# DCDmllm/AnyEdit

Measured on AMD Instinct MI355X. Metric: edited-images/sec @512x512, 50 DDIM steps, higher is better.
Workload: dtype bf16; 1 GPU; configs[1]: AnySD (SD-1.5 UNet in=8 + task embedding/expert adapters) 512x512 bf16, 50 DDIM steps, batch=4/GPU, 3-branch CFG (UNet batch 12); images_per_gpu=4, ddim_steps=50, cfg_branches=3, hip_graph=True, parallelism=dp1 (image-sharded, no data-path collective)

## Files before the change

### anyedit_amd/_lib.py

```python
import ctypes
import os

import torch

_HERE = os.path.dirname(os.path.abspath(__file__))
LIB_PATH = os.environ.get("AE_LIB_PATH") or os.path.join(_HERE, "libanyedit_hip.so")

c_void_p, c_int, c_long, c_float = ctypes.c_void_p, ctypes.c_int, ctypes.c_long, ctypes.c_float

SIGNATURES = {
    "ae_version": [],
    "ae_last_error": [],
    "ae_device_arch": [ctypes.c_char_p, c_int],
    "ae_device_info": [ctypes.POINTER(c_int), ctypes.POINTER(c_long), ctypes.POINTER(c_int)],
    "ae_gemm_bf16": [c_void_p, c_long, c_void_p, c_long, c_int, c_void_p, c_long, c_void_p, c_long, c_int, c_int, c_int,
                     c_void_p, c_void_p, c_long, c_void_p, c_long, c_int, c_int, c_int, c_void_p, c_void_p],
    "ae_conv3x3_workspace_floats": [c_int, c_int, c_int, c_int, c_int, c_int, c_int],
    "ae_conv3x3_bf16": [c_void_p, c_void_p, c_void_p, c_void_p, c_long, c_void_p, c_void_p, c_int, c_int, c_int, c_int, c_int,
                        c_int, c_int, c_int, c_void_p, c_void_p, c_int, c_void_p],
    "ae_conv3x3_up2_bf16": [c_void_p, c_void_p, c_void_p, c_void_p, c_int, c_int, c_int, c_int, c_int, c_void_p, c_void_p],
    "ae_gemm_plan": [c_int] * 8 + [ctypes.POINTER(c_int)],
    "ae_conv3x3_plan": [c_int] * 11 + [ctypes.POINTER(c_int)],
    "ae_conv3x3_up2_plan": [c_int] * 6 + [ctypes.POINTER(c_int)],
    "ae_groupnorm_rows_per_chunk": [c_int, c_int],
    "ae_groupnorm_workspace_floats": [c_int, c_int, c_int, c_int],
    "ae_groupnorm_nhwc_bf16": [c_void_p, c_void_p, c_int, c_void_p, c_void_p, c_void_p, c_int, c_int, c_int, c_int, c_float,
                               c_int, c_void_p, c_void_p, c_void_p, c_void_p, c_void_p, c_void_p],
    "ae_layernorm_bf16": [c_void_p, c_void_p, c_void_p, c_void_p, c_int, c_int, c_float, c_void_p],
    "ae_attn_fwd_bf16": [c_void_p, c_void_p, c_void_p, c_void_p, c_int, c_int, c_int, c_int, c_int,
                         c_long, c_long, c_long, c_long, c_long, c_long, c_long, c_long, c_long, c_long, c_long, c_long,
                         c_float, c_void_p, c_void_p, c_int, c_int, c_void_p, c_void_p, c_int,
                         c_void_p, c_void_p, c_int, c_long, c_long, c_long, c_long, c_long, c_long, c_void_p, c_void_p, c_void_p,
                         c_void_p],
    "ae_attn_bwd_bf16": [c_void_p] * 10 + [c_int] * 5 + [c_long] * 21 + [c_float, c_void_p, c_int, c_void_p, c_void_p],
    "ae_attn_bwd_workspace_floats": [c_int] * 5,
    "ae_groupnorm_bwd_workspace_floats": [c_int, c_int, c_int, c_int],
    "ae_groupnorm_bwd_nhwc_bf16": [c_void_p, c_void_p, c_int, c_void_p, c_void_p, c_void_p, c_void_p, c_void_p, c_int, c_int, c_int,
                                   c_int, c_float, c_int, c_void_p, c_void_p, c_void_p, c_int, c_void_p],
    "ae_layernorm_bwd_bf16": [c_void_p, c_void_p, c_void_p, c_void_p, c_void_p, c_int, c_int, c_float, c_int, c_void_p],
    "ae_layernorm_param_grad_f32": [c_void_p, c_void_p, c_void_p, c_void_p, c_void_p, c_int, c_int, c_void_p],
    "ae_add_bf16": [c_void_p, c_void_p, c_void_p, c_long, c_void_p],
    "ae_axpy_bf16": [c_void_p, c_void_p, c_float, c_void_p, c_long, c_void_p],
    "ae_geglu_fwd_bf16": [c_void_p, c_void_p, c_long, c_int, c_void_p],
    "ae_geglu_bwd_bf16": [c_void_p, c_void_p, c_void_p, c_long, c_int, c_void_p],
    "ae_sumpool2x2_bf16": [c_void_p, c_void_p, c_int, c_int, c_int, c_int, c_void_p],
    "ae_colsum_bf16_f32": [c_void_p, c_void_p, c_int, c_int, c_long, c_void_p],
    "ae_mse_grad_f32": [c_void_p, c_void_p, c_void_p, c_long, c_float, c_void_p],
    "ae_adamw_f32": [c_void_p, c_void_p, c_void_p, c_void_p, c_long, c_float, c_float, c_float, c_float, c_float, c_int, c_float,
                     c_void_p],
    "ae_rowsum_f32": [c_void_p, c_void_p, c_int, c_long, c_void_p],
    "ae_scatter_add_rows_f32": [c_void_p, c_void_p, c_void_p, c_int, c_int, c_int, c_void_p],
    "ae_attn_fp8_workspace_bytes": [c_int, c_int, c_int, c_int, c_int],
    "ae_attn_fwd_fp8": [c_void_p, c_void_p, c_void_p, c_void_p, c_int, c_int, c_int, c_int, c_int] + [c_long] * 12 +
                       [c_float, c_void_p, c_void_p, c_int, c_int, c_void_p, c_long, c_void_p],
    "ae_ln_gemm_supported": [c_int, c_int, c_int, c_int],
    "ae_ln_gemm_bf16": [c_void_p, c_long, c_void_p, c_long, c_void_p, c_long, c_int, c_int, c_int, c_void_p, c_void_p, c_long, c_void_p, c_void_p,
                        c_float, c_int, c_void_p, c_void_p],
    "ae_gemm_ln_plan": [c_int, c_int, c_int, c_int, c_int],
    "ae_ff_fused_supported": [c_int, c_int, c_int],
    "ae_ff_fused_bf16": [c_void_p, c_long, c_void_p, c_void_p, c_float, c_void_p, c_long, c_void_p, c_void_p, c_void_p, c_void_p, c_long,
                         c_void_p, c_long, c_void_p, c_void_p, c_long, c_void_p, c_void_p, c_long, c_int, c_int, c_int, c_void_p],
    "ae_gemm_ln_bf16": [c_void_p, c_long, c_void_p, c_long, c_void_p, c_long, c_int, c_int, c_int, c_void_p, c_void_p, c_long, c_int, c_void_p,
                        c_void_p, c_int, c_void_p, c_float, c_void_p],
    "ae_task_gate_bwd": [c_void_p, c_void_p, c_void_p, c_void_p, c_int, c_int, c_int, c_void_p, c_void_p],
    "ae_task_gate_wgrad": [c_void_p, c_void_p, c_void_p, c_void_p, c_void_p, c_int, c_int, c_int, c_int, c_void_p, c_void_p, c_void_p],
    "ae_expert_kv_fwd": [c_void_p, c_void_p, c_void_p, c_void_p, c_int, c_int, c_int, c_int, c_int, c_void_p],
    "ae_expert_kv_dgrad_slices": [c_int],
    "ae_expert_kv_dgrad": [c_void_p, c_void_p, c_void_p, c_void_p, c_int, c_int, c_int, c_int, c_int, c_void_p, c_void_p],
    "ae_expert_kv_wgrad": [c_void_p, c_void_p, c_void_p, c_void_p, c_int, c_int, c_int, c_int, c_int, c_void_p],
    "ae_transpose_last2": [c_void_p, c_void_p, c_int, c_int, c_int, c_int, c_int, c_int, c_void_p],
    "ae_concat_channels_bf16": [c_void_p, c_int, c_void_p, c_int, c_void_p, c_long, c_void_p],
    "ae_im2col3x3_c8_bf16": [c_void_p, c_void_p, c_int, c_int, c_int, c_void_p],
    "ae_split_channels_bf16": [c_void_p, c_int, c_int, c_void_p, c_void_p, c_long, c_int, c_int, c_void_p],
    "ae_timestep_embedding": [c_void_p, c_void_p, c_void_p, c_void_p, c_int, c_int, c_float, c_void_p],
    "ae_ddim_step_f32": [c_void_p, c_void_p, c_void_p, c_void_p, c_void_p, c_void_p, c_long, c_int, c_float, c_float, c_float,
                         c_float, c_float, c_float, c_float, c_float, c_void_p],
# ... 121 lines not shown
```

### anyedit_amd/csrc/common.hpp

```cpp
#pragma once
#include <hip/hip_runtime.h>
#include <stdint.h>

typedef uint16_t bf16_t;
typedef __attribute__((ext_vector_type(8))) __bf16 bf16x8_t;
typedef __attribute__((ext_vector_type(4))) float f32x4;
typedef __attribute__((ext_vector_type(2))) float f32x2;
typedef __attribute__((ext_vector_type(4))) uint32_t u32x4;
typedef __attribute__((ext_vector_type(2))) uint32_t u32x2;

#define AE_OK 0
#define AE_ERR_ARG -1
#define AE_ERR_LAUNCH -2
#define AE_ERR_UNSUPPORTED -3

void ae_set_error(const char* fmt, ...);
int ae_check_launch(const char* what);
int ae_launch_colstats(const uint16_t* x, long ld, int M, int N, float* out, hipStream_t stream);

int ae_rowpanel_fold_covers(int M, int N, int K, int epilogue, int mode);
int ae_rowpanel_fold_launch(const void* A, long lda, const void* W, long ldw, void* C, long ldc, int M, int N, int K, const float* bias, const void* residual,
                            long ldr, int epilogue, float* rowstats_out, const float* ln_stats, int ln_parts, const float* ln_colsum, float ln_eps, void* stream);

#define AE_REQUIRE(cond, ...)                 \
// ... 37 lines not shown
}
__device__ __forceinline__ float erf_as_f(float z) {
    const float az = __builtin_fabsf(z);
    const float t = __builtin_amdgcn_rcpf(__builtin_fmaf(0.3275911f, az, 1.0f));
    float poly = __builtin_fmaf(1.061405429f, t, -1.453152027f);
    poly = __builtin_fmaf(poly, t, 1.421413741f);
    poly = __builtin_fmaf(poly, t, -0.284496736f);
    poly = __builtin_fmaf(poly, t, 0.254829592f);
    poly *= t;
    const float e = __builtin_amdgcn_exp2f(-1.4426950408889634f * az * az);
    const float r = __builtin_fmaf(-poly, e, 1.0f);
    return __builtin_copysignf(r, z);
}
#ifndef AE_GELU_POLY
#define AE_GELU_POLY 0
#endif
__device__ __forceinline__ float gelu_w_poly_f(float x) {
    const float ax = __builtin_fminf(__builtin_fabsf(x), 4.25f);
    const float t = __builtin_fmaf(ax * ax, 0.11072664707899094f, -1.0f);
    float p = __builtin_fmaf(0.004925727378576994f, t, -0.012811211869120598f);
    p = __builtin_fmaf(p, t, 0.017165469005703926f);
    p = __builtin_fmaf(p, t, -0.02821926586329937f);
    p = __builtin_fmaf(p, t, 0.05118509382009506f);
    p = __builtin_fmaf(p, t, -0.07870230078697205f);
    p = __builtin_fmaf(p, t, 0.11140184104442596f);
    p = __builtin_fmaf(p, t, -0.1615230143070221f);
    p = __builtin_fmaf(p, t, 0.33187076449394226f);
    return ax * p;
}
__device__ __forceinline__ float gelu_w_f(float x) {
    if (AE_GELU_POLY) return gelu_w_poly_f(x);
    const float ax = __builtin_fabsf(x);
    const float t = __builtin_amdgcn_rcpf(__builtin_fmaf(0.3275911f * 0.70710678118654752440f, ax, 1.0f));
    float poly = __builtin_fmaf(1.061405429f, t, -1.453152027f);
    poly = __builtin_fmaf(poly, t, 1.421413741f);
    poly = __builtin_fmaf(poly, t, -0.284496736f);
    poly = __builtin_fmaf(poly, t, 0.254829592f);
    poly *= t;
    const float e = __builtin_amdgcn_exp2f((-0.5f * 1.4426950408889634f) * ax * ax);
    return __builtin_fmaf(-poly, e, 1.0f);
}
#ifndef AE_GELU_OLD
#define AE_GELU_OLD 0
#endif
__device__ __forceinline__ float gelu_erf_f(float x) {
    if (AE_GELU_OLD) return 0.5f * x * (1.0f + erf_as_f(x * 0.70710678118654752440f));
    return 0.5f * __builtin_fmaf(__builtin_fabsf(x), gelu_w_f(x), x);
}
__device__ __forceinline__ float geglu_half_f(float a_half, float g) {
    if (AE_GELU_OLD) return (a_half + a_half) * gelu_erf_f(g);
    return a_half * __builtin_fmaf(__builtin_fabsf(g), gelu_w_f(g), g);
}

__device__ __forceinline__ int xcd_remap(int bid, int nblocks) {
    const int NX = 8;
    int xcd = bid % NX, j = bid / NX;
    int q = nblocks / NX, r = nblocks % NX;
    int base = (xcd < r) ? xcd * (q + 1) : r * (q + 1) + (xcd - r) * q;
    return base + j;
}

__device__ __forceinline__ void ae_dma16(__amdgpu_buffer_rsrc_t rs, int lds_byte, int voffset, int soffset = 0) {
#if defined(__HIP_DEVICE_COMPILE__)
    asm volatile("s_mov_b32 m0, %2\n\ts_nop 0\n\tbuffer_load_dwordx4 %0, %1, %3 offen lds" ::"v"(voffset), "s"(rs), "s"(lds_byte), "s"(soffset)
                 : "memory", "m0");
#endif
}

__device__ __forceinline__ float wave_reduce_sum(float v) {
#pragma unroll
    for (int o = 32; o > 0; o >>= 1) v += __shfl_xor(v, o, 64);
    return v;
}
__device__ __forceinline__ float wave_reduce_max(float v) {
#pragma unroll
    for (int o = 32; o > 0; o >>= 1) v = fmaxf(v, __shfl_xor(v, o, 64));
    return v;
}
```

### anyedit_amd/csrc/gemm_conv.hip

```cpp
#include "common.hpp"
#include <stdlib.h>
#include <string.h>
#include <type_traits>

namespace {

#ifndef AE_CONV_SPEC
#define AE_CONV_SPEC 1
#endif
#ifndef AE_XE_OCC
#define AE_XE_OCC 4
#endif
#ifndef AE_PP_LAB
#define AE_PP_LAB 0
#endif
#ifndef AE_PP_PRIO
#define AE_PP_PRIO 1
#endif
#ifndef AE_PP_DMA_FIRST
#define AE_PP_DMA_FIRST 0
#endif
constexpr int BK = 64;

enum { A_DENSE = 0, A_CONV3 = 1 };
enum { EPI_NONE = 0, EPI_GELU = 1, EPI_GEGLU = 2, EPI_SILU = 3, EPI_RELU = 4 };

struct GemmArgs {
    const bf16_t* A;
    const bf16_t* A2;
    const bf16_t* W;
    void* C;
    const float* bias;
    const bf16_t* res;
    const float* addvec;
    int M, N, K, Ksplit;
    long lda, lda2, ldw, ldc, ldr, ldav;
    int epi, out_f32, rows_per_batch;
    int H, Wd, Cin, CinPad, Ho, Wo, stride, ups;
    unsigned a_bytes, a2_bytes, w_bytes;
    int splitk;
    float* partial;
    float* colstats;
    int kmajor;
    int m_fast;
    int xe;
    float* rowstats;
    const float* ln_stats;
    const float* ln_colsum;
    int ln_parts;
    float ln_eps;
    int sub2;
};

__device__ __forceinline__ void lds_dma16(__amdgpu_buffer_rsrc_t rs, bf16_t* lds_dst, int voffset, int soffset = 0) {
#if defined(__HIP_DEVICE_COMPILE__)
    __builtin_amdgcn_raw_ptr_buffer_load_lds(rs, (__attribute__((address_space(3))) void*)lds_dst, 16, voffset, soffset, 0, 0);
#endif
}

#ifdef AE_GEMM_LAB
__device__ unsigned long long g_gemm_dbg[32];
#define GL_T(i) do { const unsigned long long t_ = __builtin_readcyclecounter(); if (lab_me) g_gemm_dbg[lab_base + (i)] += t_ - tlast; tlast = t_; } while (0)
#elif defined(AE_GEMM_TRACE)
constexpr int TR_K0 = 18, TR_T = 6;
__device__ unsigned long long g_pp_trace[8 * TR_T * 16];
#define GL_T(i) do { __builtin_amdgcn_sched_barrier(0); tr_t[(i)] = __builtin_readcyclecounter(); __builtin_amdgcn_sched_barrier(0); } while (0)
#else
#define GL_T(i)
#endif

constexpr int epilogue_passes(int FM, int bytes_per_frag_row, int lds_bytes) {
    for (int ps = 1; ps <= FM; ++ps)
        if (FM % ps == 0 && (FM / ps) * bytes_per_frag_row <= lds_bytes) return ps;
    return FM;
}

template <int BM, int BN, int AMODE, int WAVES_M = 2, int WAVES_N = 2, bool GLDS = false, int WAVES_K = 1, int STAGES = 2, bool CS = false, int LAB = 0, int WA = 0, int XE = 0>
__global__ __launch_bounds__(64 * WAVES_M * WAVES_N * WAVES_K, (XE == 2 && BM == 128 && BN == 128 && STAGES == 2) ? AE_XE_OCC : 0) void gemm_kernel(const GemmArgs p) {
    static_assert(XE == 0 || (AMODE == A_DENSE && WAVES_K == 1 && !CS && GLDS), "row statistics / LayerNorm fold: dense LDS-DMA instantiations, one K group, no column statistics");
    static_assert(XE != 1 || BN / WAVES_N == 64, "row statistics are emitted per 64-column slice = one wave tile's width");
    static_assert(STAGES == 2 || (GLDS && WAVES_K == 1), "the deep LDS ring exists only for the LDS-DMA loader");
    static_assert(!WA || (GLDS && STAGES == 2 && WAVES_K == 1), "operand-ahead is a variant of the two-stage LDS-DMA pipeline");
    static_assert(WA == 0 || WA == 1 || WA == 3 || WA == 4, "WA: 0 none, 1 weights two tiles ahead (three W stages), 3 ping-pong (two wave groups one barrier apart), 4 ping-pong over an activation slab per (channel chunk, ky)");
    static_assert(WA < 3 || 64 * WAVES_M * WAVES_N * WAVES_K == 512, "the ping-pong loops pair wave w with wave w + 4 (one SIMD's two waves)");
    static_assert(WA != 4 || (AMODE == A_CONV3 && GLDS && BM % 16 == 0), "the slab loop is a 3x3-convolution loop");
    static_assert(WAVES_K == 1, "one K group per block (the two-group form is removed: DESIGN.md, \"Built, measured, removed\")");
    constexpr int NT = 64 * WAVES_M * WAVES_N * WAVES_K;
    constexpr int WM = BM / WAVES_M, WN = BN / WAVES_N;
    constexpr int FM = WM / 16, FN = WN / 16;
    constexpr int A_CH = BM * 8 / NT, B_CH = BN * 8 / NT;
    static_assert((BM * 8) % NT == 0 && (BN * 8) % NT == 0, "tile / thread-count combination not supported");
    extern __shared__ __attribute__((aligned(16))) unsigned char smem_raw[];
    bf16_t* const smem = reinterpret_cast<bf16_t*>(smem_raw);
    bf16_t* sA = smem;
    bf16_t* sB = smem + (WA >= 3 ? 3 : STAGES) * BM * BK;

#ifndef AE_WAVE_SGPR
#define AE_WAVE_SGPR 1
#endif
    const int tid = threadIdx.x, lane = tid & 63, wave = AE_WAVE_SGPR ? __builtin_amdgcn_readfirstlane(tid >> 6) : tid >> 6;
#ifdef AE_GEMM_TRACE
    const bool tr_blk = blockIdx.x == gridDim.x / 2 && WA == 3;
    unsigned long long* const tr_lds = reinterpret_cast<unsigned long long*>(smem_raw + 152 * 1024);
    int tr_kt = -1;
    unsigned long long tr_t[16];
#pragma unroll
    for (int q = 0; q < 16; ++q) tr_t[q] = 0;
#endif
#ifdef AE_GEMM_LAB
    unsigned long long tlast = __builtin_readcyclecounter();
    const bool lab_me = blockIdx.x == gridDim.x / 2 && lane == 0 && (wave == 0 || wave == 4);
    const int lab_base = wave == 0 ? 0 : 16;
#endif
    const int wk = wave / (WAVES_M * WAVES_N), wmn = wave % (WAVES_M * WAVES_N);
    const int wm = wmn / WAVES_N, wn = wmn % WAVES_N;
    const int l15 = lane & 15, lg = lane >> 4;
    const int ntn = (p.N + BN - 1) / BN, ntm = (p.M + BM - 1) / BM;
    const int ntiles = ntm * ntn;
    const int split = blockIdx.x / ntiles;
    const int py = (AMODE == A_CONV3 && p.sub2) ? split >> 1 : 0, px = (AMODE == A_CONV3 && p.sub2) ? split & 1 : 0;
    const int tile = xcd_remap(blockIdx.x % ntiles, ntiles);
    const int m0 = (p.m_fast ? tile % ntm : tile / ntn) * BM, n0 = (p.m_fast ? tile / ntm : tile % ntn) * BN;

    long a_base[A_CH];
    int a_iy[A_CH], a_ix[A_CH];
#pragma unroll
    for (int i = 0; i < A_CH; ++i) {
        const int row = (tid + i * NT) >> 3;
        const int m = m0 + row;
        const int mc = min(m, p.M - 1);
        if (AMODE == A_DENSE) {
            a_base[i] = (long)mc;
            a_iy[i] = a_ix[i] = 0;
        } else {
            const int hw = p.Ho * p.Wo;
            const int b = mc / hw, rem = mc - b * hw;
            const int oy = rem / p.Wo, ox = rem - oy * p.Wo;
            a_base[i] = (long)b * p.H * p.Wd;
            a_iy[i] = (m < p.M) ? oy * p.stride - 1 : -100000;
            a_ix[i] = ox * p.stride - 1;
        }
    }
    long b_base[B_CH];
#pragma unroll
    for (int i = 0; i < B_CH; ++i) {
        const int row = (tid + i * NT) >> 3;
        b_base[i] = (long)min(n0 + row, p.N - 1) * p.ldw;
    }

    const __amdgpu_buffer_rsrc_t rsA = __builtin_amdgcn_make_buffer_rsrc(const_cast<bf16_t*>(p.A), 0, (int)p.a_bytes, 0x00020000);
    const __amdgpu_buffer_rsrc_t rsA2 = __builtin_amdgcn_make_buffer_rsrc(const_cast<bf16_t*>(p.A2 ? p.A2 : p.A), 0, (int)(p.A2 ? p.a2_bytes : 0u), 0x00020000);
    const __amdgpu_buffer_rsrc_t rsW = __builtin_amdgcn_make_buffer_rsrc(const_cast<bf16_t*>(p.W) + ((AMODE == A_CONV3 && p.sub2) ? (long)split * p.N * p.ldw : 0L), 0, (int)p.w_bytes, 0x00020000);
    constexpr int OOB = (int)0x80000000;
    int fa_off[A_CH], fa2_off[A_CH], fb_off[B_CH];
    unsigned fa_mask[A_CH];
#pragma unroll
    for (int i = 0; i < A_CH; ++i) {
        const int id = tid + i * NT, row = id >> 3;
        const int c = GLDS ? ((id & 7) ^ (row & 7)) : (id & 7);
        const int m = m0 + row;
        fa_mask[i] = 0u;
        if (AMODE == A_DENSE) {
            fa_off[i] = (m < p.M) ? (int)((long)m * p.lda * 2) + c * 16 : OOB;
            fa2_off[i] = (m < p.M) ? (int)((long)m * p.lda2 * 2) + c * 16 : OOB;
        } else {
            fa2_off[i] = OOB;
            const int hw = p.Ho * p.Wo;
            const int mc = min(m, p.M - 1);
            const int b = mc / hw, rem = mc - b * hw;
            const int oy = rem / p.Wo, ox = rem - oy * p.Wo;
            const int iy0 = oy * p.stride - 1, ix0 = ox * p.stride - 1;
            fa_off[i] = (int)(((long)(b * p.H + iy0) * p.Wd + ix0) * p.Cin + c * 8) * 2;
            const int Hv = p.ups ? 2 * p.H : p.H, Wv = p.ups ? 2 * p.Wd : p.Wd;
            if (m < p.M) {
#pragma unroll
// ... 1033 lines not shown
struct Plan { int tile, splitk; };
Plan make_plan(int M, int N, int K, bool can_split) {
    const int t = pick_tile(M, N);
    const int kt = (K + BK - 1) / BK;
    static const int force_s = getenv("AE_GEMM_SPLITK") ? atoi(getenv("AE_GEMM_SPLITK")) : 0;
    static const int t320_split = getenv("AE_CONV_T320_SPLITK") ? atoi(getenv("AE_CONV_T320_SPLITK")) : 3;
    if (t320_split && can_split && N % 320 == 0 && M % 192 == 0 && force_s <= 0) {
        const long t192 = (long)(M / 192) * (N / 320);
        if (t192 >= 32 && t192 <= (t320_split == 2 ? 64 : (t320_split == 3 && kt < 180 ? 64 : 128))) {
            int s = (int)(256 / t192);
            if (s > 8) s = 8;
            while (s > 1 && kt / s < 16) --s;
            if (s >= 2) return {4, s};
        }
    }
    if (!can_split || kt < 32 || t == 0 || t == 3) return {t, 1};
    const long t128 = (long)((M + 127) / 128) * ((N + 127) / 128);
    const double waste128 = (double)(((N + 127) / 128) * 128) / (double)N;
    if (waste128 <= 1.10 && t128 < 256) {
        int s = force_s > 0 ? force_s : (int)((480 + t128 - 1) / t128);
        static const int smax = getenv("AE_CONV_SPLIT_MAX") ? atoi(getenv("AE_CONV_SPLIT_MAX")) : 8;
        if (s > smax) s = smax;
        if (s > kt / 8) s = kt / 8;
        if (s >= 2) return {0, s};
    }
    return {t, 1};
}

template <typename Kern>
int launch_kernel(Kern kern, unsigned grid, int threads, size_t lds, hipStream_t stream, const GemmArgs& a, const char* what) {
    if (lds > 64 * 1024) {
        static const void* done[32];
        static int ndone = 0;
        const void* fn = reinterpret_cast<const void*>(kern);
        bool seen = false;
        for (int i = 0; i < ndone; ++i) seen |= done[i] == fn;
        if (!seen) {
            if (hipFuncSetAttribute(fn, hipFuncAttributeMaxDynamicSharedMemorySize, (int)lds) != hipSuccess) {
                ae_set_error("hipFuncSetAttribute(MaxDynamicSharedMemorySize=%zu) failed", lds);
                return AE_ERR_LAUNCH;
            }
            if (ndone < 32) done[ndone++] = fn;
        }
    }
    hipLaunchKernelGGL(kern, dim3(grid), dim3(threads), lds, stream, a);
    return ae_check_launch(what);
}

struct PlanReport {
    int BM, BN, AMODE, WAVES_M, WAVES_N, GLDS, WAVES_K, STAGES, CS, LAB, WA, XE;
    int grid, threads, lds, splitk;
    int reduce, colstats;
    int rowpanel;
};
#define AE_PLAN_INTS 19
static_assert(sizeof(PlanReport) == AE_PLAN_INTS * sizeof(int), "PlanReport is the int array of anyedit_hip.h");

void* const kQueryPtr = reinterpret_cast<void*>(uintptr_t(256));
float* const kQueryF32 = reinterpret_cast<float*>(uintptr_t(256));
int plan_out(int rc, const PlanReport& r, int* plan) {
    if (!rc) memcpy(plan, &r, sizeof r);
    return rc;
}

struct LaunchCtx { const GemmArgs& a; hipStream_t stream; const char* what; PlanReport* report; };

template <int BM, int BN, int AMODE, int WAVES_M = 2, int WAVES_N = 2, bool GLDS = false, int WAVES_K = 1, int STAGES = 2, bool CS = false, int LAB = 0, int WA = 0, int XE = 0>
int run_tile(const LaunchCtx& c, long grid, size_t lds) {
    constexpr int threads = 64 * WAVES_M * WAVES_N * WAVES_K;
    if (c.report) {
        *c.report = PlanReport{BM, BN, AMODE, WAVES_M, WAVES_N, GLDS, WAVES_K, STAGES, CS, LAB, WA, XE, (int)grid, threads, (int)lds, c.a.splitk, 0, 0, 0};
        return 0;
    }
    return launch_kernel(gemm_kernel<BM, BN, AMODE, WAVES_M, WAVES_N, GLDS, WAVES_K, STAGES, CS, LAB, WA, XE>, (unsigned)grid, threads, lds, c.stream, c.a, c.what);
}

template <int BM, int BN, int AMODE, int WAVES_M, int WAVES_N>
int run_plain(const LaunchCtx& c, bool glds, long grid) {
    const size_t lds = (size_t)2 * (BM + BN) * BK * sizeof(bf16_t);
    return glds ? run_tile<BM, BN, AMODE, WAVES_M, WAVES_N, true>(c, grid, lds) : run_tile<BM, BN, AMODE, WAVES_M, WAVES_N, false>(c, grid, lds);
}

template <int AMODE>
int launch(const GemmArgs& a_in, hipStream_t stream, PlanReport* report = nullptr, int split_tile = 0) {
    GemmArgs a = a_in;
    static const int mfast_env = getenv("AE_GEMM_MFAST") ? atoi(getenv("AE_GEMM_MFAST")) : -1;
    a.m_fast = mfast_env >= 0 ? mfast_env : (AMODE == A_CONV3 ? (9L * a.N >= 8L * a.M) : ((long)a.N >= 3L * a.M)) ? 1 : 0;
    const int cand[4][2] = {{128, 128}, {128, 64}, {64, 64}, {128, 160}};
    static const int t160 = getenv("AE_GEMM_T160") ? atoi(getenv("AE_GEMM_T160")) : 1;
    int pick = a.splitk > 1 ? 0 : pick_tile(a.M, a.N);
    static const int force_tile = getenv("AE_GEMM_TILE") ? atoi(getenv("AE_GEMM_TILE")) : -1;
    if (force_tile >= 0 && force_tile <= 2 && a.splitk <= 1) pick = force_tile;
    if (pick == 3 && (!t160 || AMODE == A_DENSE || a.epi == EPI_GEGLU || a.splitk > 1)) pick = 1;
    const int kt_block = ((a.K + BK - 1) / BK + a.splitk - 1) / a.splitk;
    const bool conv = AMODE == A_CONV3;
    const char* what = conv ? "ae_conv3x3_bf16" : "ae_gemm_bf16";
    const LaunchCtx lc{a, stream, what, report};
    static const int glds_env = getenv("AE_GEMM_GLDS") ? atoi(getenv("AE_GEMM_GLDS")) : 1;
    const bool glds = glds_env && (conv ? (a.Cin == a.CinPad) : (a.K % BK == 0 && (!a.A2 || a.Ksplit % BK == 0)));
    if (conv && a.kmajor && !glds) { ae_set_error("%s: the chunk-major K order exists only in the LDS-DMA loader (AE_GEMM_GLDS=0 is set)", what); return AE_ERR_UNSUPPORTED; }
    auto lds_of = [](int bm, int bn, int st) { return (size_t)st * (bm + bn) * BK * sizeof(bf16_t); };
    auto lds_wa = [](int bm, int bn) { return (size_t)(2 * bm + 3 * bn) * BK * sizeof(bf16_t); };
#ifdef AE_GEMM_TRACE
    auto lds_aa = [](int bm, int bn) { return (size_t)(3 * bm + 2 * bn) * BK * sizeof(bf16_t) + 8192; };
#else
    auto lds_aa = [](int bm, int bn) { return (size_t)(3 * bm + 2 * bn) * BK * sizeof(bf16_t); };
#endif
    int rc = 0;

    static const int t320 = getenv("AE_GEMM_T320") ? atoi(getenv("AE_GEMM_T320")) : 11;
    bool done = false;
    bool xe_done = false;
    const bool cs_epi_ok = a.colstats && a.epi != EPI_GEGLU && !a.out_f32 && a.splitk <= 1 && a.N % 8 == 0 && a.ldc % 8 == 0 &&
                           (!a.res || (a.ldr % 8 == 0 && (reinterpret_cast<uintptr_t>(a.res) & 15) == 0));
    bool cs_done = false;
#ifdef AE_GEMM_ABLATE
    static const int lab_abl = getenv("AE_GEMM_ABL") ? atoi(getenv("AE_GEMM_ABL")) : 0;
#endif
    const bool slab_ok = conv && a.kmajor && a.stride == 1 && !a.ups && a.Cin == a.CinPad && a.H == a.Ho && a.Wd == a.Wo && a.Wd % 16 == 0 && 192 % a.Wd == 0 &&
                         192 / a.Wd <= a.H + 1 &&
                         (a.splitk <= 1 || kt_block % 9 == 0);
    const size_t lds_slab = (size_t)2 * ((192 + 192 / 16 + 1 + 7) / 8) * 1024 + (size_t)2 * 320 * BK * sizeof(bf16_t);
    if (conv && a.splitk > 1 && glds && split_tile == 4) {
        const long t = (long)(a.M / 192) * (a.N / 320) * a.splitk;
        if constexpr (AMODE == A_CONV3) {
            if (slab_ok) rc = run_tile<192, 320, A_CONV3, 2, 4, true, 1, 2, false, 0, 4>(lc, t, lds_slab);
            else if (!a.ups) rc = run_tile<192, 320, A_CONV3, 2, 4, true, 1, 2, false, 0, 3>(lc, t, lds_aa(192, 320));
            else rc = run_tile<192, 320, A_CONV3, 2, 4, true>(lc, t, lds_of(192, 320, 2));
        }
        done = true;
    }
    if (!done && t320 && glds && a.splitk <= 1 && a.N % 320 == 0 && ((conv && (t320 & 1)) || (!conv && a.epi == EPI_GEGLU && a.K >= 640 && (t320 & 2)) || (!conv && a.epi == EPI_GEGLU && a.K < 640 && a.K >= 320 && (t320 & 4)) ||
                                                                     (!conv && a.epi != EPI_GEGLU && a.K >= 640 && (t320 & 8)))) {
        const long t = (long)((a.M + 191) / 192) * (a.N / 320);
        const double fill = (double)t / (double)(((t + 255) / 256) * 256) * ((double)a.M / (double)(((a.M + 191) / 192) * 192));
        static const int t320_xe = getenv("AE_GEMM_T320_XE") ? atoi(getenv("AE_GEMM_T320_XE")) : 1;
        const long t128x = (long)((a.M + 127) / 128) * ((a.N + 127) / 128);
        const bool xe_tail = t320_xe && !conv && a.xe == 2 && a.epi != EPI_GEGLU && fill >= 0.74 && fill < 0.85 &&
                             (double)t128x / (double)(((t128x + 511) / 512) * 512) <= 0.72;
        if (fill >= 0.85 || xe_tail) {
// ... 171 lines not shown
    if (rc) return rc;
    if (a.xe) {
        PlanReport r;
        rc = launch<A_DENSE>(a, nullptr, &r);
        if (rc) return rc;
    }
    return launch<A_DENSE>(a, (hipStream_t)stream);
}
}

extern "C" int ae_gemm_bf16(const void* A, long lda, const void* A2, long lda2, int Ksplit, const void* W, long ldw,
                            void* C, long ldc, int M, int N, int K, const float* bias, const void* residual, long ldr,
                            const float* addvec, long addvec_ld, int rows_per_batch, int epilogue, int out_f32, float* colstats, void* stream) {
    return gemm_entry(A, lda, A2, lda2, Ksplit, W, ldw, C, ldc, M, N, K, bias, residual, ldr, addvec, addvec_ld, rows_per_batch, epilogue, out_f32, colstats, LnExtras{}, stream);
}

extern "C" int ae_gemm_ln_bf16(const void* A, long lda, const void* W, long ldw, void* C, long ldc, int M, int N, int K, const float* bias,
                               const void* residual, long ldr, int epilogue, float* rowstats_out, const float* ln_stats, int ln_parts,
                               const float* ln_colsum, float ln_eps, void* stream) {
    AE_REQUIRE((rowstats_out != nullptr) != (ln_stats != nullptr), "ae_gemm_ln_bf16: exactly one of rowstats_out (emit) and ln_stats (consume) must be given");
    AE_REQUIRE(A && W && C && M > 0 && N > 0 && K > 0, "ae_gemm_ln_bf16: null pointer or empty shape");
    {
        const int rc = ae_rowpanel_fold_launch(A, lda, W, ldw, C, ldc, M, N, K, bias, residual, ldr, epilogue, rowstats_out, ln_stats, ln_parts, ln_colsum, ln_eps, stream);
        if (rc != AE_ERR_UNSUPPORTED) return rc;
    }
    LnExtras x;
    x.rowstats_out = rowstats_out; x.ln_stats = ln_stats; x.ln_colsum = ln_colsum; x.ln_parts = ln_parts; x.ln_eps = ln_eps;
    return gemm_entry(A, lda, nullptr, 0, 0, W, ldw, C, ldc, M, N, K, bias, residual, ldr, nullptr, 0, 0, epilogue, 0, nullptr, x, stream);
}

extern "C" int ae_gemm_plan(int M, int N, int K, int epilogue, int Ksplit, int out_f32, int colstats, int ln_mode, int* plan) {
    AE_REQUIRE(plan && ln_mode >= 0 && ln_mode <= 2, "ae_gemm_plan: null plan or LN mode %d outside 0..2", ln_mode);
    AE_REQUIRE(M > 0 && N > 0 && K > 0 && K % 8 == 0 && epilogue >= EPI_NONE && epilogue <= EPI_RELU, "ae_gemm_plan: bad shape or epilogue");
    PlanReport r{};
    r.rowpanel = ln_mode ? ae_rowpanel_fold_covers(M, N, K, epilogue, ln_mode) : 0;
    if (r.rowpanel) return plan_out(0, r, plan);
    AE_REQUIRE(ln_mode != 1 || N <= 1280, "ae_gemm_plan: the consumer of row statistics sums up to 20 slices per row (N = %d)", N);
    void* const p = kQueryPtr;
    float* const f = kQueryF32;
    LnExtras x;
    if (ln_mode == 1) x.rowstats_out = f;
    if (ln_mode == 2) { x.ln_stats = f; x.ln_colsum = f; x.ln_parts = K / 64; }
    GemmArgs a;
    const int rc = gemm_args(a, p, K, Ksplit > 0 ? p : nullptr, K, Ksplit, p, K, p, epilogue == EPI_GEGLU ? N / 2 : N, M, N, K, ln_mode == 2 ? f : nullptr, nullptr, 0,
                             nullptr, 0, 0, epilogue, out_f32, colstats ? f : nullptr, x);
    return plan_out(rc ? rc : launch<A_DENSE>(a, nullptr, &r), r, plan);
}

extern "C" int ae_gemm_ln_plan(int M, int N, int K, int epilogue, int mode) {
    int plan[AE_PLAN_INTS];
    return (mode == 1 || mode == 2) && ae_gemm_plan(M, N, K, epilogue, 0, 0, 0, mode, plan) == 0 ? 1 : 0;
}

namespace {
int launch_sub2(GemmArgs a, hipStream_t stream, PlanReport* report = nullptr) {
    const LaunchCtx lc{a, stream, "ae_conv3x3_up2_bf16", report};
    a.m_fast = (9L * a.N >= 8L * a.M) ? 1 : 0;
    const bool cs = a.colstats != nullptr;
    int rc;
    const long t192 = (a.M % 192 == 0 && a.N % 320 == 0) ? (long)(a.M / 192) * (a.N / 320) * 4 : 0;
    if (t192 > 0 && (double)t192 / (double)(((t192 + 255) / 256) * 256) >= 0.85) {
        const size_t lds = (size_t)(3 * 192 + 2 * 320) * BK * sizeof(bf16_t);
        if (cs) rc = run_tile<192, 320, A_CONV3, 2, 4, true, 1, 2, true, 0, 3>(lc, t192, lds);
        else rc = run_tile<192, 320, A_CONV3, 2, 4, true, 1, 2, false, 0, 3>(lc, t192, lds);
    } else {
        const unsigned grid = (unsigned)((long)((a.M + 127) / 128) * ((a.N + 127) / 128) * 4);
        const size_t lds = (size_t)(2 * 128 + 3 * 128) * BK * sizeof(bf16_t);
        if (cs) rc = run_tile<128, 128, A_CONV3, 4, 2, true, 1, 2, true, 0, 1>(lc, grid, lds);
        else rc = run_tile<128, 128, A_CONV3, 4, 2, true, 1, 2, false, 0, 1>(lc, grid, lds);
    }
    return rc;
}
}

namespace {
int up2_args(GemmArgs& a, const void* x, const void* w4, const float* bias, void* y, int B, int H, int W, int Cin, int Cout, float* colstats) {
    AE_REQUIRE(x && w4 && y, "ae_conv3x3_up2_bf16: null pointer");
    AE_REQUIRE(B > 0 && H > 0 && W > 0, "ae_conv3x3_up2_bf16: bad shape B=%d H=%d W=%d", B, H, W);
    AE_REQUIRE(Cin % 64 == 0 && Cout % 8 == 0, "ae_conv3x3_up2_bf16: Cin %% 64 == 0 (whole K tiles per tap) and Cout %% 8 == 0 (row-contiguous stores), got %d -> %d", Cin, Cout);
    AE_REQUIRE(aligned16(x) && aligned16(w4) && aligned16(y), "ae_conv3x3_up2_bf16: pointers must be 16-byte aligned");
    if (colstats) AE_REQUIRE((H * W) % 32 == 0 && (reinterpret_cast<uintptr_t>(colstats) & 15) == 0, "ae_conv3x3_up2_bf16: column statistics are kept per 32-row slab of a sample and parity: H * W = %d must be a multiple of 32", H * W);
    AE_REQUIRE((long)B * H * W * Cin * 2 < (1L << 31) && (long)Cout * 4 * Cin * 2 < (1L << 31) && (long)B * 4 * H * W < (1L << 31), "ae_conv3x3_up2_bf16: operands must be smaller than 2 GiB");
    a = GemmArgs{};
    a.A = (const bf16_t*)x; a.A2 = nullptr; a.W = (const bf16_t*)w4; a.C = y;
    a.bias = bias; a.res = nullptr; a.addvec = nullptr;
    a.M = B * H * W; a.N = Cout; a.K = 4 * Cin; a.Ksplit = a.K;
    a.lda = 0; a.lda2 = 0; a.ldw = 4L * Cin; a.ldc = Cout; a.ldr = Cout; a.ldav = Cout;
    a.epi = EPI_NONE; a.out_f32 = 0; a.rows_per_batch = H * W;
    a.H = H; a.Wd = W; a.Cin = Cin; a.CinPad = Cin; a.Ho = H; a.Wo = W; a.stride = 1; a.ups = 0;
    a.a_bytes = (unsigned)((long)B * H * W * Cin * 2); a.a2_bytes = 0u; a.w_bytes = (unsigned)((long)Cout * 4 * Cin * 2);
    a.splitk = 1; a.partial = nullptr; a.colstats = colstats; a.kmajor = 0; a.sub2 = 1;
    return 0;
}
}

extern "C" int ae_conv3x3_up2_bf16(const void* x, const void* w4, const float* bias, void* y, int B, int H, int W, int Cin, int Cout, float* colstats, void* stream) {
    GemmArgs a;
    const int rc = up2_args(a, x, w4, bias, y, B, H, W, Cin, Cout, colstats);
    return rc ? rc : launch_sub2(a, (hipStream_t)stream);
}

extern "C" int ae_conv3x3_up2_plan(int B, int H, int W, int Cin, int Cout, int colstats, int* plan) {
    AE_REQUIRE(plan, "ae_conv3x3_up2_plan: null plan");
    GemmArgs a;
    PlanReport r{};
    const int rc = up2_args(a, kQueryPtr, kQueryPtr, nullptr, kQueryPtr, B, H, W, Cin, Cout, colstats ? kQueryF32 : nullptr);
    return plan_out(rc ? rc : launch_sub2(a, nullptr, &r), r, plan);
}

extern "C" long ae_conv3x3_workspace_floats(int B, int H, int W, int Cin, int Cout, int stride, int upsample2x) {
// ... 64 lines not shown
```

### anyedit_amd/ops.py

```python
import torch

import collections
import ctypes
import os
import threading

from ._lib import lib, check as _check

BF16 = torch.bfloat16
EPI_NONE, EPI_GELU, EPI_GEGLU, EPI_SILU, EPI_RELU = 0, 1, 2, 3, 4


def _s():
    return torch.cuda.current_stream().cuda_stream


def _p(t):
    return None if t is None else t.data_ptr()


_live = threading.local()


def _tmp(t):
# ... 91 lines not shown
                for j in range(2):
                    acc = torch.zeros(cout, cin, dtype=torch.float32, device=w.device)
                    for ky in sets[(py, i)]:
                        for kx in sets[(px, j)]:
                            acc = acc + w32[:, :, ky, kx]
                    out[2 * py + px, :, 2 * i + j] = acc
    return out


_UP2_SUBPIXEL = os.environ.get("AE_UP2_SUBPIXEL", "1") != "0"


def up2_subpixel_ok(Cin, Cout, H, W, want_stats):
    return _UP2_SUBPIXEL and Cin % 64 == 0 and Cout % 8 == 0 and (not want_stats or (H * W) % 32 == 0) and not (_TAPE is not None and _TAPE.active)


def conv3x3_up2(x, w4, bias, B, H, W, out=None, colstats=None):
    _chk(x, BF16, "conv3x3_up2.x", 2)
    _chk(w4, BF16, "conv3x3_up2.w4", 3)
    Cin, Cout = x.shape[1], w4.shape[1]
    if x.shape[0] != B * H * W or not x.is_contiguous():
        raise ValueError(f"conv3x3_up2: x must be contiguous [B*H*W, Cin] = [{B * H * W}, Cin], got {tuple(x.shape)}")
    if tuple(w4.shape) != (4, Cout, 4 * Cin) or not w4.is_contiguous():
        raise ValueError(f"conv3x3_up2: packed weight must be a contiguous [4, Cout, {4 * Cin}] tensor, got {tuple(w4.shape)}")
    if out is None:
        out = torch.empty(B * 4 * H * W, Cout, dtype=BF16, device=x.device)
    if colstats is not None:
        _chk(colstats, torch.float32, "conv3x3_up2.colstats", 3)
        if tuple(colstats.shape) != (B * 4 * H * W // 32, Cout, 2) or not colstats.is_contiguous() or (H * W) % 32:
            raise ValueError(f"conv3x3_up2: colstats must be a contiguous [{B * 4 * H * W // 32}, {Cout}, 2] fp32 buffer (H * W % 32 == 0)")
    check(lib.ae_conv3x3_up2_bf16(_p(x), _p(w4), _p(bias), _p(out), B, H, W, Cin, Cout, _p(colstats), _s()), "ae_conv3x3_up2_bf16")
    return out, 2 * H, 2 * W


_STEM_IM2COL = os.environ.get("AE_STEM_IM2COL", "1") != "0"


def stem_im2col_ok(Cin, stride, upsample2x):
    return _STEM_IM2COL and Cin == 8 and stride == 1 and not upsample2x and not (_TAPE is not None and _TAPE.active)


def im2col3x3_c8(x, B, H, W):
    _chk(x, BF16, "im2col3x3_c8.x", 2)
    if tuple(x.shape) != (B * H * W, 8) or not x.is_contiguous():
        raise ValueError(f"im2col3x3_c8: x must be contiguous [{B * H * W}, 8], got {tuple(x.shape)}")
    y = torch.empty(B * H * W, 128, dtype=BF16, device=x.device)
    check(lib.ae_im2col3x3_c8_bf16(_p(x), _p(y), B, H, W, _s()), "ae_im2col3x3_c8_bf16")
    return y


_CONV_KMAJOR = int(os.environ.get("AE_CONV_KMAJOR", "2"))


Plan = collections.namedtuple("Plan", "BM BN AMODE WAVES_M WAVES_N GLDS WAVES_K STAGES CS LAB WA XE grid threads lds splitk reduce colstats rowpanel")
_PLANS = {}


def _plan(query, *args):
    key = (query,) + args
    if key not in _PLANS:
        buf = (ctypes.c_int * len(Plan._fields))()
        _PLANS[key] = Plan(*buf) if getattr(lib, query)(*args, buf) == 0 else None
    return _PLANS[key]


def gemm_plan(M, N, K, epilogue=EPI_NONE, Ksplit=0, out_f32=False, colstats=False, ln_mode=0):
    return _plan("ae_gemm_plan", M, N, K, epilogue, Ksplit, int(out_f32), int(colstats), ln_mode)


def conv_plan(B, H, W, Cin, Cout, stride=1, upsample2x=0, out_f32=False, colstats=False, k_order=0):
    return _plan("ae_conv3x3_plan", B, H, W, Cin, Cout, stride, int(upsample2x), int(out_f32), 1, int(colstats), int(k_order))


def up2_plan(B, H, W, Cin, Cout, colstats=False):
    return _plan("ae_conv3x3_up2_plan", B, H, W, Cin, Cout, int(colstats))


def plan_label(p):
    return f"{p.BM}x{p.BN}" + (",ring3" if p.STAGES == 3 else "") + (",splitK" if p.splitk > 1 else "")


def conv_k_order(M, Cin, Cout, stride=1, upsample2x=False):
    if _CONV_KMAJOR == 0 or upsample2x or Cin % 64 != 0 or (_TAPE is not None and _TAPE.active):
        return 0
    p = conv_plan(M, 1, 1, Cin, Cout, stride)
    if p is None or not p.GLDS:
        return 0
    if _CONV_KMAJOR == 3:
        return 1
    label = plan_label(p)
    if _CONV_KMAJOR == 4:
        return 1 if label in ("192x320", "128x128") else 0
    return 1 if (label == "192x320" or (_CONV_KMAJOR >= 2 and label == "192x320,splitK")) else 0


def pack_geglu(w, b):
    inner = w.shape[0] // 2
    assert inner % 16 == 0
    a, g = w[:inner], w[inner:]
    wp = torch.stack([a.reshape(inner // 16, 16, -1), g.reshape(inner // 16, 16, -1)], dim=1).reshape(2 * inner, -1)
    bp = torch.stack([b[:inner].reshape(-1, 16), b[inner:].reshape(-1, 16)], dim=1).reshape(-1)
    return wp.detach().to(BF16).contiguous(), bp.detach().float().contiguous()


def pack_ff2_fused(w2):
    C, H = w2.shape
    assert C == 320 and H % 32 == 0
    dev = w2.device
    i = torch.arange(C, device=dev)
    i5 = i & 31
    col = 32 * (i >> 5) + 8 * ((i5 & 15) >> 2) + 4 * (i5 >> 4) + (i5 & 3)
    pos = torch.arange(4, device=dev)
# ... 2477 lines not shown
```

### include/anyedit_hip.h

```cpp
#ifndef ANYEDIT_HIP_H
#define ANYEDIT_HIP_H

#ifdef __cplusplus
extern "C" {
#endif

#define AE_OK 0
#define AE_ERR_ARG (-1)
#define AE_ERR_LAUNCH (-2)
#define AE_ERR_UNSUPPORTED (-3)

#define AE_EPI_NONE 0
#define AE_EPI_GELU 1
#define AE_EPI_GEGLU 2
#define AE_EPI_SILU 3
#define AE_EPI_RELU 4

int ae_version(void);
const char* ae_last_error(void);
int ae_device_arch(char* buf, int n);
int ae_device_info(int* cus, long* hbm_bytes, int* clock_khz);

int ae_gemm_bf16(const void* A, long lda, const void* A2, long lda2, int Ksplit, const void* W, long ldw, void* C, long ldc,
                 int M, int N, int K, const float* bias, const void* residual, long ldr, const float* addvec, long addvec_ld,
                 int rows_per_batch, int epilogue, int out_f32, float* colstats, void* stream);

int ae_ln_gemm_supported(int M, int N, int K, int epilogue);
int ae_ln_gemm_bf16(const void* A, long lda, const void* W, long ldw, void* C, long ldc, int M, int N, int K, const float* bias,
                    const void* residual, long ldr, const float* ln_gamma, const float* ln_beta, float ln_eps, int epilogue,
                    float* colstats , void* stream);

int ae_gemm_ln_plan(int M, int N, int K, int epilogue, int mode);
int ae_gemm_ln_bf16(const void* A, long lda, const void* W, long ldw, void* C, long ldc, int M, int N, int K, const float* bias,
                    const void* residual, long ldr, int epilogue, float* rowstats_out, const float* ln_stats, int ln_parts,
                    const float* ln_colsum, float ln_eps, void* stream);

int ae_ff_fused_supported(int M, int C, int H);
int ae_ff_fused_bf16(const void* X, long ldx, const float* ln_gamma, const float* ln_beta, float ln_eps, const void* W1, long ldw1, const float* b1,
                     const void* W2img, const float* b2, const void* residual, long ldr, const void* W3, long ldw3, const float* b3,
                     const void* residual3, long ldr3, float* colstats, void* Y, long ldy, int M, int C, int H, void* stream);

long ae_conv3x3_workspace_floats(int B, int H, int W, int Cin, int Cout, int stride, int upsample2x);
int ae_conv3x3_bf16(const void* x, const void* w, const float* bias, const float* addvec, long addvec_ld, const void* residual,
                    void* y, int B, int H, int W, int Cin, int Cout, int stride, int upsample2x, int out_f32, float* workspace,
                    float* colstats , int k_order, void* stream);

int ae_conv3x3_up2_bf16(const void* x, const void* w4, const float* bias, void* y, int B, int H, int W, int Cin, int Cout,
                        float* colstats, void* stream);

#define AE_PLAN_INTS 19
int ae_gemm_plan(int M, int N, int K, int epilogue, int Ksplit, int out_f32, int colstats, int ln_mode, int* plan);
int ae_conv3x3_plan(int B, int H, int W, int Cin, int Cout, int stride, int upsample2x, int out_f32, int workspace, int colstats, int k_order,
                    int* plan);
int ae_conv3x3_up2_plan(int B, int H, int W, int Cin, int Cout, int colstats, int* plan);

int ae_groupnorm_rows_per_chunk(int HW, int C);
long ae_groupnorm_workspace_floats(int B, int HW, int C, int groups);
int ae_groupnorm_nhwc_bf16(const void* x, const void* x2, int C1, const float* gamma, const float* beta, void* y, int B, int HW,
                           int C, int groups, float eps, int act, float* workspace, int* counters, float* stat_out,
                           const float* colstats, const float* colstats2, void* stream);

int ae_layernorm_bf16(const void* x, const float* gamma, const float* beta, void* y, int M, int C, float eps, void* stream);

int ae_attn_fwd_bf16(const void* q, const void* k, const void* v, void* out, int B, int H, int Nq, int Nk, int D,
                     long q_sb, long q_sh, long q_sn, long k_sb, long k_sh, long k_sn, long v_sb, long v_sh, long v_sn,
                     long o_sb, long o_sh, long o_sn, float scale, const float* rel_h, const float* rel_w, int kH, int kW,
                     const unsigned char* key_mask, const float* out_scale, int accumulate, const void* k2, const void* v2,
                     int Nk2, long k2_sb, long k2_sh, long k2_sn, long v2_sb, long v2_sh, long v2_sn, const float* scale2,
                     float* lse, float* lse2, void* stream);
long ae_attn_fp8_workspace_bytes(int B, int H, int Nq, int Nk, int D);
int ae_attn_fwd_fp8(const void* q, const void* k, const void* v, void* out, int B, int H, int Nq, int Nk, int D, long q_sb, long q_sh,
                    long q_sn, long k_sb, long k_sh, long k_sn, long v_sb, long v_sh, long v_sn, long o_sb, long o_sh, long o_sn,
                    float scale, const float* rel_h, const float* rel_w, int kH, int kW, void* workspace, long workspace_bytes,
                    void* stream);
long ae_attn_bwd_workspace_floats(int B, int H, int Nq, int Nk, int D);
int ae_attn_bwd_bf16(const void* q, const void* k, const void* v, const void* dout, const void* out, const float* lse, float* delta, void* dq,
                     void* dk, void* dv, int B, int H, int Nq, int Nk, int D, long q_sb, long q_sh, long q_sn, long k_sb,
                     long k_sh, long k_sn, long v_sb, long v_sh, long v_sn, long o_sb, long o_sh, long o_sn, long dq_sb,
                     long dq_sh, long dq_sn, long dk_sb, long dk_sh, long dk_sn, long dv_sb, long dv_sh, long dv_sn,
                     float scale, const float* out_scale, int accumulate_dq, float* workspace, void* stream);
long ae_groupnorm_bwd_workspace_floats(int B, int HW, int C, int groups);
int ae_groupnorm_bwd_nhwc_bf16(const void* x, const void* x2, int C1, const float* gamma, const float* beta, const void* dy,
                               void* dx, void* dx2, int B, int HW, int C, int groups, float eps, int act, float* workspace,
                               int* counters, const float* stat_in, int accumulate, void* stream);
int ae_layernorm_bwd_bf16(const void* x, const float* gamma, const void* dy, void* dx, float* row_stat, int M, int C, float eps,
                          int accumulate, void* stream);
int ae_layernorm_param_grad_f32(const void* x, const void* dy, const float* row_stat, float* dgamma, float* dbeta, int M, int C,
                                void* stream);
int ae_add_bf16(const void* a, const void* b, void* y, long n, void* stream);
int ae_axpy_bf16(const void* a, const void* b, float alpha, void* y, long n, void* stream);
int ae_geglu_fwd_bf16(const void* h, void* y, long M, int F, void* stream);
int ae_geglu_bwd_bf16(const void* h, const void* dy, void* dh, long M, int F, void* stream);
int ae_sumpool2x2_bf16(const void* x, void* y, int B, int H, int W, int C, void* stream);
int ae_colsum_bf16_f32(const void* x, float* out, int M, int N, long ld, void* stream);
int ae_mse_grad_f32(const float* pred, const float* target, float* out, long n, float loss_scale, void* stream);
int ae_adamw_f32(float* param, const float* grad, float* exp_avg, float* exp_avg_sq, long n, float lr, float beta1, float beta2,
                 float eps, float weight_decay, int step, float grad_scale, void* stream);
int ae_rowsum_f32(const float* x, float* out, int rows, long n, void* stream);
int ae_scatter_add_rows_f32(const float* src, const int* code, float* dst, int B, int D, int n_rows, void* stream);
int ae_task_gate_bwd(const float* probs, const int* top1, const float* dgate, const float* Wg, int B, int Dt, int E, float* dte,
                     void* stream);
int ae_task_gate_wgrad(const float* probs, const int* top1, const float* dgate, const float* task_emb, const long* edit_code, int B,
                       int n_tasks, int Dt, int E, float* dWg, float* dbg, void* stream);

int ae_expert_kv_fwd(const void* x, const float* W, const int* experts, void* y, int B, int T, int N, int Dc, int E, void* stream);
int ae_expert_kv_dgrad_slices(int N);
int ae_expert_kv_dgrad(const void* dy, const float* W, const int* experts, void* dx, int B, int T, int N, int Dc, int E, float* partial,
// ... 172 lines not shown
```

Before: 6.569 edited-images/sec.

## Add grouped tile rasterization for GEMM kernels to improve L2 reuse

Replaces the one-dimensional m-fast/n-fast tile ordering with a grouped (swizzled) raster that walks tiles in gm x gn windows after the XCD remap. A host-side cost model picks the group shape from tile counts, LDS size and split copies. By default (mode 1) grouping applies only to non-conv, non-split GEMMs; other launches keep the 1-D order. It adds a few integer divisions per block and a runtime override, and risks worse locality when the heuristic misjudges the window.

New measurement: 6.570 edited-images/sec, median of 2. Within noise of the previous version (+0.0%).

```diff
diff --git a/anyedit_amd/_lib.py b/anyedit_amd/_lib.py
--- a/anyedit_amd/_lib.py
+++ b/anyedit_amd/_lib.py
@@ -22,6 +22,8 @@
     "ae_gemm_plan": [c_int] * 8 + [ctypes.POINTER(c_int)],
     "ae_conv3x3_plan": [c_int] * 11 + [ctypes.POINTER(c_int)],
     "ae_conv3x3_up2_plan": [c_int] * 6 + [ctypes.POINTER(c_int)],
+    "ae_gemm_set_raster": [c_int],
+    "ae_tile_raster_map": [c_int] * 5 + [ctypes.POINTER(c_int), ctypes.POINTER(c_int)],
     "ae_groupnorm_rows_per_chunk": [c_int, c_int],
     "ae_groupnorm_workspace_floats": [c_int, c_int, c_int, c_int],
     "ae_groupnorm_nhwc_bf16": [c_void_p, c_void_p, c_int, c_void_p, c_void_p, c_void_p, c_int, c_int, c_int, c_int, c_float,
diff --git a/anyedit_amd/csrc/common.hpp b/anyedit_amd/csrc/common.hpp
--- a/anyedit_amd/csrc/common.hpp
+++ b/anyedit_amd/csrc/common.hpp
@@ -113,12 +113,26 @@
     return a_half * __builtin_fmaf(__builtin_fabsf(g), gelu_w_f(g), g);
 }
 
-__device__ __forceinline__ int xcd_remap(int bid, int nblocks) {
+__host__ __device__ __forceinline__ int xcd_remap(int bid, int nblocks) {
     const int NX = 8;
     int xcd = bid % NX, j = bid / NX;
     int q = nblocks / NX, r = nblocks % NX;
     int base = (xcd < r) ? xcd * (q + 1) : r * (q + 1) + (xcd - r) * q;
     return base + j;
+}
+
+struct TileCoord { int tm, tn; };
+__host__ __device__ __forceinline__ TileCoord tile_raster(int bid, int ntm, int ntn, int gm, int gn, int order) {
+    const int t = xcd_remap(bid, ntm * ntn);
+    const int na = order ? ntn : ntm, nb = order ? ntm : ntn, ga = order ? gn : gm, gb = order ? gm : gn;
+    const int band_tiles = ga * nb;
+    const int band = t / band_tiles, r = t - band * band_tiles;
+    const int rest = na - band * ga, h = rest < ga ? rest : ga;
+    const int group_tiles = h * gb;
+    const int g = r / group_tiles, r2 = r - g * group_tiles;
+    const int q = r2 / h;
+    const int a = band * ga + (r2 - q * h), b = g * gb + q;
+    return order ? TileCoord{b, a} : TileCoord{a, b};
 }
 
 __device__ __forceinline__ void ae_dma16(__amdgpu_buffer_rsrc_t rs, int lds_byte, int voffset, int soffset = 0) {
diff --git a/anyedit_amd/csrc/gemm_conv.hip b/anyedit_amd/csrc/gemm_conv.hip
--- a/anyedit_amd/csrc/gemm_conv.hip
+++ b/anyedit_amd/csrc/gemm_conv.hip
@@ -1,6 +1,7 @@
 #include "common.hpp"
 #include <stdlib.h>
 #include <string.h>
+#include <atomic>
 #include <type_traits>
 
 namespace {
@@ -42,7 +43,7 @@
     float* partial;
     float* colstats;
     int kmajor;
-    int m_fast;
+    int gm, gn, rorder;
     int xe;
     float* rowstats;
     const float* ln_stats;
@@ -119,8 +120,8 @@
     const int ntiles = ntm * ntn;
     const int split = blockIdx.x / ntiles;
     const int py = (AMODE == A_CONV3 && p.sub2) ? split >> 1 : 0, px = (AMODE == A_CONV3 && p.sub2) ? split & 1 : 0;
-    const int tile = xcd_remap(blockIdx.x % ntiles, ntiles);
-    const int m0 = (p.m_fast ? tile % ntm : tile / ntn) * BM, n0 = (p.m_fast ? tile / ntm : tile % ntn) * BN;
+    const TileCoord tile = tile_raster(blockIdx.x % ntiles, ntm, ntn, p.gm, p.gn, p.rorder);
+    const int m0 = tile.tm * BM, n0 = tile.tn * BN;
 
     long a_base[A_CH];
     int a_iy[A_CH], a_ix[A_CH];
@@ -1260,8 +1261,9 @@
     int grid, threads, lds, splitk;
     int reduce, colstats;
     int rowpanel;
+    int gm, gn, order;
 };
-#define AE_PLAN_INTS 19
+#define AE_PLAN_INTS 22
 static_assert(sizeof(PlanReport) == AE_PLAN_INTS * sizeof(int), "PlanReport is the int array of anyedit_hip.h");
 
 void* const kQueryPtr = reinterpret_cast<void*>(uintptr_t(256));
@@ -1273,14 +1275,52 @@
 
 struct LaunchCtx { const GemmArgs& a; hipStream_t stream; const char* what; PlanReport* report; };
 
+std::atomic<int> g_raster_set{-1};
+int raster_mode() {
+    static const int env = getenv("AE_GEMM_RASTER") ? atoi(getenv("AE_GEMM_RASTER")) : 1;
+    const int s = g_raster_set.load(std::memory_order_relaxed);
+    return s >= 0 ? s : env;
+}
+
+struct Raster { int gm, gn, order; };
+Raster choose_raster(const GemmArgs& a, int BM, int BN, bool conv, size_t lds) {
+    const int ntm = (a.M + BM - 1) / BM, ntn = (a.N + BN - 1) / BN;
+    static const int mfast_env = getenv("AE_GEMM_MFAST") ? atoi(getenv("AE_GEMM_MFAST")) : -1;
+    const bool m_fast = mfast_env >= 0 ? mfast_env != 0 : (conv ? (9L * a.N >= 8L * a.M) : ((long)a.N >= 3L * a.M));
+    const Raster one_d = m_fast ? Raster{ntm, 1, 0} : Raster{1, ntn, 0};
+    const int mode = raster_mode();
+    const int copies = a.sub2 ? 4 : a.splitk > 1 ? a.splitk : 1;
+    const bool grouped_class = !conv && copies == 1;
+    if (mode <= 0 || mfast_env >= 0 || (mode == 1 && !grouped_class)) return one_d;
+    int window = 32 * (lds > 80 * 1024 ? 1 : 2) / copies;
+    const int run = ntm * ntn / 8;
+    if (window > run) window = run;
+    if (window < 1) window = 1;
+    const long cA = conv ? BM : 3L * BM, cW = 3L * BN;
+    Raster best{1, 1, 0};
+    long best_cost = 0, best_tiles = 0;
+    for (int gm = ntm < window ? ntm : window; gm >= 1; --gm) {
+        int gn = window / gm;
+        if (gn > ntn) gn = ntn;
+        const long cost = gm * cA + gn * cW, tiles = (long)gm * gn;
+        if (!best_tiles || cost * best_tiles < best_cost * tiles) { best = Raster{gm, gn, 0}; best_cost = cost; best_tiles = tiles; }
+    }
+    if (best.gn == ntn) return Raster{1, ntn, 0};
+    if (best.gm == ntm) return Raster{ntm, 1, 0};
+    return best;
+}
+
 template <int BM, int BN, int AMODE, int WAVES_M = 2, int WAVES_N = 2, bool GLDS = false, int WAVES_K = 1, int STAGES = 2, bool CS = false, int LAB = 0, int WA = 0, int XE = 0>
 int run_tile(const LaunchCtx& c, long grid, size_t lds) {
     constexpr int threads = 64 * WAVES_M * WAVES_N * WAVES_K;
+    const Raster rs = choose_raster(c.a, BM, BN, AMODE == A_CONV3, lds);
     if (c.report) {
-        *c.report = PlanReport{BM, BN, AMODE, WAVES_M, WAVES_N, GLDS, WAVES_K, STAGES, CS, LAB, WA, XE, (int)grid, threads, (int)lds, c.a.splitk, 0, 0, 0};
+        *c.report = PlanReport{BM, BN, AMODE, WAVES_M, WAVES_N, GLDS, WAVES_K, STAGES, CS, LAB, WA, XE, (int)grid, threads, (int)lds, c.a.splitk, 0, 0, 0, rs.gm, rs.gn, rs.order};
         return 0;
     }
-    return launch_kernel(gemm_kernel<BM, BN, AMODE, WAVES_M, WAVES_N, GLDS, WAVES_K, STAGES, CS, LAB, WA, XE>, (unsigned)grid, threads, lds, c.stream, c.a, c.what);
+    GemmArgs a = c.a;
+    a.gm = rs.gm; a.gn = rs.gn; a.rorder = rs.order;
+    return launch_kernel(gemm_kernel<BM, BN, AMODE, WAVES_M, WAVES_N, GLDS, WAVES_K, STAGES, CS, LAB, WA, XE>, (unsigned)grid, threads, lds, c.stream, a, c.what);
 }
 
 template <int BM, int BN, int AMODE, int WAVES_M, int WAVES_N>
@@ -1291,9 +1331,7 @@
 
 template <int AMODE>
 int launch(const GemmArgs& a_in, hipStream_t stream, PlanReport* report = nullptr, int split_tile = 0) {
-    GemmArgs a = a_in;
-    static const int mfast_env = getenv("AE_GEMM_MFAST") ? atoi(getenv("AE_GEMM_MFAST")) : -1;
-    a.m_fast = mfast_env >= 0 ? mfast_env : (AMODE == A_CONV3 ? (9L * a.N >= 8L * a.M) : ((long)a.N >= 3L * a.M)) ? 1 : 0;
+    const GemmArgs& a = a_in;
     const int cand[4][2] = {{128, 128}, {128, 64}, {64, 64}, {128, 160}};
     static const int t160 = getenv("AE_GEMM_T160") ? atoi(getenv("AE_GEMM_T160")) : 1;
     int pick = a.splitk > 1 ? 0 : pick_tile(a.M, a.N);
@@ -1571,10 +1609,26 @@
     return (mode == 1 || mode == 2) && ae_gemm_plan(M, N, K, epilogue, 0, 0, 0, mode, plan) == 0 ? 1 : 0;
 }
 
+extern "C" int ae_gemm_set_raster(int mode) {
+    AE_REQUIRE(mode >= -1 && mode <= 2, "ae_gemm_set_raster: mode %d outside -1..2", mode);
+    g_raster_set.store(mode, std::memory_order_relaxed);
+    return 0;
+}
+
+extern "C" int ae_tile_raster_map(int ntm, int ntn, int gm, int gn, int order, int* tm, int* tn) {
+    AE_REQUIRE(tm && tn && ntm > 0 && ntn > 0 && (long)ntm * ntn < (1L << 30), "ae_tile_raster_map: null output or bad tile grid %d x %d", ntm, ntn);
+    AE_REQUIRE(gm >= 1 && gm <= ntm && gn >= 1 && gn <= ntn && (order == 0 || order == 1), "ae_tile_raster_map: group %d x %d (order %d) outside the %d x %d grid", gm, gn, order, ntm, ntn);
+    for (int b = 0; b < ntm * ntn; ++b) {
+        const TileCoord t = tile_raster(b, ntm, ntn, gm, gn, order);
+        tm[b] = t.tm;
+        tn[b] = t.tn;
+    }
+    return 0;
+}
+
 namespace {
 int launch_sub2(GemmArgs a, hipStream_t stream, PlanReport* report = nullptr) {
     const LaunchCtx lc{a, stream, "ae_conv3x3_up2_bf16", report};
-    a.m_fast = (9L * a.N >= 8L * a.M) ? 1 : 0;
     const bool cs = a.colstats != nullptr;
     int rc;
     const long t192 = (a.M % 192 == 0 && a.N % 320 == 0) ? (long)(a.M / 192) * (a.N / 320) * 4 : 0;
diff --git a/anyedit_amd/ops.py b/anyedit_amd/ops.py
--- a/anyedit_amd/ops.py
+++ b/anyedit_amd/ops.py
@@ -167,12 +167,20 @@
 _CONV_KMAJOR = int(os.environ.get("AE_CONV_KMAJOR", "2"))
 
 
-Plan = collections.namedtuple("Plan", "BM BN AMODE WAVES_M WAVES_N GLDS WAVES_K STAGES CS LAB WA XE grid threads lds splitk reduce colstats rowpanel")
+Plan = collections.namedtuple("Plan", "BM BN AMODE WAVES_M WAVES_N GLDS WAVES_K STAGES CS LAB WA XE grid threads lds splitk reduce colstats rowpanel gm gn order")
 _PLANS = {}
+_RASTER = -1
+
+
+def set_gemm_raster(mode):
+    global _RASTER
+    prev, _RASTER = _RASTER, int(mode)
+    check(lib.ae_gemm_set_raster(_RASTER), "ae_gemm_set_raster")
+    return prev
 
 
 def _plan(query, *args):
-    key = (query,) + args
+    key = (query, _RASTER) + args
     if key not in _PLANS:
         buf = (ctypes.c_int * len(Plan._fields))()
         _PLANS[key] = Plan(*buf) if getattr(lib, query)(*args, buf) == 0 else None
diff --git a/include/anyedit_hip.h b/include/anyedit_hip.h
--- a/include/anyedit_hip.h
+++ b/include/anyedit_hip.h
@@ -48,11 +48,14 @@
 int ae_conv3x3_up2_bf16(const void* x, const void* w4, const float* bias, void* y, int B, int H, int W, int Cin, int Cout,
                         float* colstats, void* stream);
 
-#define AE_PLAN_INTS 19
+#define AE_PLAN_INTS 22
 int ae_gemm_plan(int M, int N, int K, int epilogue, int Ksplit, int out_f32, int colstats, int ln_mode, int* plan);
 int ae_conv3x3_plan(int B, int H, int W, int Cin, int Cout, int stride, int upsample2x, int out_f32, int workspace, int colstats, int k_order,
                     int* plan);
 int ae_conv3x3_up2_plan(int B, int H, int W, int Cin, int Cout, int colstats, int* plan);
+
+int ae_tile_raster_map(int ntm, int ntn, int gm, int gn, int order, int* tm, int* tn);
+int ae_gemm_set_raster(int mode);
 
 int ae_groupnorm_rows_per_chunk(int HW, int C);
 long ae_groupnorm_workspace_floats(int B, int HW, int C, int groups);
```
